# PaoPaoRobot/ygz-slam

Measured on NVIDIA H100. Metric: tracked frames/sec, higher is better.
Workload: dtype u8+f32+f64

## Files before the change

ygz_slam_b200/csrc/align.cu:

```cuda
#include <algorithm>
#include <cstdlib>
#include <mutex>

#include <cooperative_groups.h>

#include "common.cuh"
#include "se3.cuh"
#include "track.cuh"

namespace ygzb {

namespace {

struct LevelImg {
    const uint8_t* d;
    int w, h, pitch;
};

__device__ __forceinline__ LevelImg level_img(const uint8_t* pyr, size_t slot_stride, int slot, const Geometry& g, int L) {
    return LevelImg{pyr + (size_t)slot * slot_stride + g.lv[L].off, g.lv[L].w, g.lv[L].h, g.lv[L].pitch};
}

__device__ void inverse3f(const float H[3][3], float inv[3][3]) {
#define COF(i, j) (H[(i + 1) % 3][(j + 1) % 3] * H[(i + 2) % 3][(j + 2) % 3] - H[(i + 1) % 3][(j + 2) % 3] * H[(i + 2) % 3][(j + 1) % 3])
// ... 524 lines not shown
    cluster.sync();
    if (rank == 0 && tid == 0) {
        const SE3d Tref = se3_from_mat(a.T_ref + 12 * (size_t)prob);
        se3_to_mat(se3_mul(s_T, Tref), a.T_cur + 12 * (size_t)prob);
        a.n_meas_out[prob] = (int32_t)(s_last_nmeas / 16);
    }
}


constexpr int kSA2Threads = 256;
constexpr int kSA2Terms = 21 + 6 + 1;

struct SA2Feat {
    float patch[16], gdx[16], gdy[16];
    double FJ[12];
    double G[3];
    double xyz[3];
    float u, v;
    int ui, vi;
    int state;
    int pad;
};

__device__ __forceinline__ double sa2_rcp(double x) {
    double r;
    asm("rcp.approx.ftz.f64 %0, %1;" : "=d"(r) : "d"(x));
    r = fma(r, fma(-x, r, 1.0), r);
    r = fma(r, fma(-x, r, 1.0), r);
    return r;
}

__device__ bool ldlt_solve6_fast(const double H[6][6], const double b[6], double x[6]) {
    double L[6][6], D[6], rD[6];
    for (int j = 0; j < 6; ++j) {
        double d = H[j][j];
        for (int k = 0; k < j; ++k) d -= L[j][k] * L[j][k] * D[k];
        D[j] = d;
        if (!(fabs(d) > 0)) return false;
        rD[j] = sa2_rcp(fabs(d));
        if (d < 0) rD[j] = -rD[j];
        L[j][j] = 1;
        for (int i = j + 1; i < 6; ++i) {
            double s = H[i][j];
            for (int k = 0; k < j; ++k) s -= L[i][k] * L[j][k] * D[k];
            L[i][j] = s * rD[j];
        }
    }
    double y[6];
    for (int i = 0; i < 6; ++i) {
        double s = b[i];
        for (int k = 0; k < i; ++k) s -= L[i][k] * y[k];
        y[i] = s;
    }
    for (int i = 0; i < 6; ++i) y[i] *= rD[i];
    for (int i = 5; i >= 0; --i) {
        double s = y[i];
        for (int k = i + 1; k < 6; ++k) s -= L[k][i] * x[k];
        x[i] = s;
    }
    return true;
}

// ... 233 lines not shown
    b.cur_slot[j] = job.cur_slot;
    b.n_cand[j] = 0;
    b.c_off[j] = j * b.cap;
    if (j == 0) b.c_off[b.J] = b.J * b.cap;
    if (b.prev) {
        const int r = 2 * job.stream + st.ref_cur[job.stream];
        b.ref_slot[j] = b.job_ref_slot[j];
        b.offsets[j] = j * st.ref_cap;
        if (j == 0) b.offsets[b.J] = b.J * st.ref_cap;
        b.in_off[j] = r * st.ref_cap;
        b.n_feat[j] = st.ref_n[r];
        for (int c = 0; c < 12; ++c) b.T_ref[12 * (size_t)j + c] = b.T_cur[12 * (size_t)j + c] = st.ref_T[12 * (size_t)r + c];
        return;
    }
    const int e = job.stream * st.R + job.entry[job.n_local - 1];
    b.ref_slot[j] = st.kf_slot[e];
    b.offsets[j] = j * st.cells;
    if (j == 0) b.offsets[b.J] = b.J * st.cells;
    b.in_off[j] = e * st.cells;
    b.n_feat[j] = st.kf_n[e];
    for (int c = 0; c < 12; ++c) b.T_ref[12 * (size_t)j + c] = b.T_cur[12 * (size_t)j + c] = (c == 0 || c == 5 || c == 10) ? 1.0 : 0.0;
}

__global__ void track_compose_kernel(TrackStore st, TrackBatch b) {
    const int j = blockIdx.x * blockDim.x + threadIdx.x;
    if (j >= b.J) return;
    const ygzb_track_job job = b.jobs[j];
    if (b.prev) {
        for (int c = 0; c < 12; ++c) b.T_aligned[12 * (size_t)j + c] = b.T_cur[12 * (size_t)j + c];
        return;
    }
    const double* Tk = st.kf_T + 12 * (size_t)(job.stream * st.R + job.entry[job.n_local - 1]);
    const SE3d Trel = se3_from_mat(b.T_cur + 12 * (size_t)j), Tref = se3_from_mat(Tk);
    se3_to_mat(se3_mul(Trel, Tref), b.T_cur + 12 * (size_t)j);
    for (int c = 0; c < 12; ++c) {
        b.T_ref[12 * (size_t)j + c] = Tk[c];
        b.T_aligned[12 * (size_t)j + c] = b.T_cur[12 * (size_t)j + c];
    }
}

__global__ void track_motion_kernel(TrackStore st, TrackBatch b) {
    const int j = blockIdx.x * blockDim.x + threadIdx.x;
    if (j >= b.J) return;
    const ygzb_track_job job = b.jobs[j];
    const double* Tc = b.T_cur + 12 * (size_t)j;
    double inv_ref[12], tcr[12], lg[6];
    mat34_inv(b.T_ref + 12 * (size_t)j, inv_ref);
    mat34_mul(Tc, inv_ref, tcr);
    se3_log(se3_from_mat(tcr), lg);
    double nrm = 0;
    for (int k = 0; k < 6; ++k) nrm += lg[k] * lg[k];
    b.aligned[j] = sqrt(nrm) <= 0.2 ? 1 : 0;
    for (int k = 0; k < job.n_local; ++k) {
        double inv_k[12];
        mat34_inv(st.kf_T + 12 * (size_t)(job.stream * st.R + job.entry[k]), inv_k);
        mat34_mul(Tc, inv_k, b.rel + 12 * ((size_t)j * kTrackMaxLocal + k));
    }
}

__global__ void __launch_bounds__(128) track_project_kernel(const uint8_t* __restrict__ pyr, size_t slot_stride, Geometry g, CamF cam,
                                                            TrackStore st, TrackBatch b) {
    const int j = blockIdx.y, c = blockIdx.x * blockDim.x + threadIdx.x;
    if (c >= b.cap) return;
    const size_t at = (size_t)j * b.cap + c;
    b.cand_ok[at] = 0;
    if (!b.aligned[j]) return;
    const ygzb_track_job job = b.jobs[j];
    const int k = c / st.cells, f = c - k * st.cells;
    if (k >= job.n_local) return;
    const int e = job.stream * st.R + job.entry[k];
    if (f >= st.kf_n[e]) return;
    const double* X = st.kf_pw + 3 * ((size_t)e * st.cells + f);
    const double* T = b.T_cur + 12 * (size_t)j;
    const double x = T[0] * X[0] + T[1] * X[1] + T[2] * X[2] + T[3];
    const double y = T[4] * X[0] + T[5] * X[1] + T[6] * X[2] + T[7];
    const double z = T[8] * X[0] + T[9] * X[1] + T[10] * X[2] + T[11];
    double u = st.fx * x / z + st.cx, v = st.fy * y / z + st.cy;
    if (!(z > 0 && u >= 20 && u < st.W - 20 && v >= 20 && v < st.H - 20)) return;
    atomicAdd(&b.n_cand[j], 1);
    const double eye[12] = {1, 0, 0, 0, 0, 1, 0, 0, 0, 0, 1, 0};
// ... 15 lines not shown
        if (lane >= o) v += u;
    }
    if (lane == 31) s_w[warp] = v;
    __syncthreads();
    if (warp == 0) {
        int w = s_w[lane];
#pragma unroll
        for (int o = 1; o < 32; o <<= 1) {
            const int u = __shfl_up_sync(0xFFFFFFFFu, w, o);
            if (lane >= o) w += u;
        }
        s_w[lane] = w;
        if (lane == 31) s_w[32] = w;
    }
    __syncthreads();
    const int out = v + (warp ? s_w[warp - 1] : 0);
    *total = s_w[32];
    __syncthreads();
    return out;
}

__global__ void __launch_bounds__(1024) track_compact_kernel(TrackStore st, TrackBatch b) {
    __shared__ int s_scan[33];
    __shared__ int s_carry;
    const int j = blockIdx.x, tid = threadIdx.x;
    const ygzb_track_job job = b.jobs[j];
    const int total = job.n_local * st.cells;
    if (tid == 0) s_carry = 0;
    __syncthreads();
    for (int base = 0; base < total; base += 1024) {
        const int c = base + tid;
        const int flag = (c < total && b.cand_ok[(size_t)j * b.cap + c]) ? 1 : 0;
        int chunk_total;
        const int incl = block_scan_1024(flag, s_scan, &chunk_total);
        if (flag) {
            const size_t dst = (size_t)j * b.cap + s_carry + incl - 1;
            const int k = c / st.cells, f = c - k * st.cells;
            const size_t fe = (size_t)(job.stream * st.R + job.entry[k]) * st.cells + f;
            b.c_src[dst] = c;
            b.c_px[2 * dst] = b.cand_px[2 * ((size_t)j * b.cap + c)];
            b.c_px[2 * dst + 1] = b.cand_px[2 * ((size_t)j * b.cap + c) + 1];
            b.c_pw[3 * dst] = st.kf_pw[3 * fe];
            b.c_pw[3 * dst + 1] = st.kf_pw[3 * fe + 1];
            b.c_pw[3 * dst + 2] = st.kf_pw[3 * fe + 2];
        }
        __syncthreads();
        if (tid == 0) s_carry += chunk_total;
        __syncthreads();
    }
    if (tid == 0) b.c_cnt[j] = s_carry;
}

}

size_t sparse_align2_scratch_bytes(int n_problems, int max_features) { return (size_t)n_problems * max_features * sizeof(SA2Feat); }
size_t sparse_align_ws_doubles(int n_problems) { return (size_t)n_problems * 2 * kSparseCluster * (kNormalTerms + 1); }

int launch_align2d(ygzb_frames* f, int n, const int32_t* d_slot, const uint8_t* d_level, const uint8_t* d_ref_border,
                   const uint8_t* d_ref, int n_iter, double* d_uv, uint8_t* d_ok) {
    ygzb_ctx* ctx = f->ctx;
    if (n <= 0) return YGZB_OK;
    ProfScope ps(ctx, kStageAlign2D);
    align2d_kernel<<<(n + 127) / 128, 128, 0, ctx->stream>>>(f->d_pyr, ctx->slot_stride, ctx->geo, n, d_slot, d_level, d_ref_border,
                                                             d_ref, n_iter, d_uv, d_ok);
    YGZB_LAUNCHED(ctx);
    return YGZB_OK;
}

int launch_align1d(ygzb_frames* f, int n, const int32_t* d_slot, const uint8_t* d_level, const float* d_dir, const uint8_t* d_ref_border,
                   const uint8_t* d_ref, int n_iter, double* d_uv, uint8_t* d_ok, double* d_hinv) {
    ygzb_ctx* ctx = f->ctx;
    if (n <= 0) return YGZB_OK;
    ProfScope ps(ctx, kStageAlign2D);
// ... 145 lines not shown
    a.max_level = 2;
    a.min_level = 0;
    a.n_iter = 30;
    a.eps = 1e-6;
    a.n_meas_out = b.n_meas;
    a.iters_out = nullptr;
    a.ref_patch = b.ref_patch;
    a.gdx = b.gdx;
    a.gdy = b.gdy;
    a.frame_jac = b.frame_jac;
    a.visible = b.visible;
    a.ws = b.sparse_ws;
    a.feat_scratch = nullptr;
    a.feat_stride = 0;
    if (gen1) return launch_sparse_align1(ctx, a, b.J, sparse_cluster);
    return launch_sparse_align2(ctx, a, b.J, sparse_cluster, b.sa2_scratch, sparse_align2_scratch_bytes(1, feat_cap));
}

int launch_track_chain_mid(ygzb_frames* f, const TrackStore& st, const TrackBatch& b) {
    ygzb_ctx* ctx = f->ctx;
    if (b.J <= 0) return YGZB_OK;
    {
        ProfScope ps(ctx, kStageOther);
        track_compose_kernel<<<(b.J + 63) / 64, 64, 0, ctx->stream>>>(st, b);
        YGZB_LAUNCHED(ctx);
    }
    {
        ProfScope ps(ctx, kStageOther);
        track_motion_kernel<<<(b.J + 63) / 64, 64, 0, ctx->stream>>>(st, b);
        YGZB_LAUNCHED(ctx);
    }
    {
        const CamF cam{ctx->prm.fx, ctx->prm.fy, ctx->prm.cx, ctx->prm.cy};
        ProfScope ps(ctx, kStageProjectAlign);
        track_project_kernel<<<dim3((unsigned)((b.cap + 127) / 128), (unsigned)b.J), 128, 0, ctx->stream>>>(f->d_pyr, ctx->slot_stride, ctx->geo,
                                                                                                          cam, st, b);
        YGZB_LAUNCHED(ctx);
    }
    {
        ProfScope ps(ctx, kStageOther);
        track_compact_kernel<<<(unsigned)b.J, 1024, 0, ctx->stream>>>(st, b);
        YGZB_LAUNCHED(ctx);
    }
    return YGZB_OK;
}

}
```

ygz_slam_b200/csrc/ba.cu:

```cuda
#include <algorithm>
#include <cstdlib>
#include <cstring>
#include <exception>
#include <mutex>
#include <utility>
#include <vector>

#include <cooperative_groups.h>

#include "ba2.cuh"
#include "common.cuh"
#include "se3.cuh"
#include "track.cuh"

namespace ygzb {

namespace {

constexpr int kBAThreads = 256;
constexpr int kMaxFreePoses = 16;
constexpr int kMaxPoses = 64;

struct BAArgs {
    const int32_t *kf_off, *pt_off, *obs_off;
// ... 846 lines not shown
    double* T_cw;
    uint8_t* inlier;
    double* depth;
    int32_t* n_inlier;
    uint8_t* enable;
    double* ws;
    float fx, fy, cx, cy;
    int stage_k;
};

constexpr int kPoseThreads = 256;
constexpr int kPoseCluster = 8;
constexpr int kPoseRed = 32;

__device__ bool cholesky6(double A[36], double y[6]) {
    double rd[6];
#pragma unroll
    for (int j = 0; j < 6; ++j) {
        double d = A[j * 6 + j];
#pragma unroll
        for (int k = 0; k < j; ++k) d -= A[j * 6 + k] * A[j * 6 + k] * A[k * 6 + k];
        if (!(d > 0)) return false;
        A[j * 6 + j] = d;
        rd[j] = 1.0 / d;
#pragma unroll
        for (int i = j + 1; i < 6; ++i) {
            double s = A[i * 6 + j];
#pragma unroll
            for (int k = 0; k < j; ++k) s -= A[i * 6 + k] * A[j * 6 + k] * A[k * 6 + k];
            A[i * 6 + j] = s * rd[j];
        }
    }
#pragma unroll
    for (int i = 0; i < 6; ++i) {
        double s = y[i];
#pragma unroll
        for (int k = 0; k < i; ++k) s -= A[i * 6 + k] * y[k];
        y[i] = s;
    }
#pragma unroll
    for (int i = 0; i < 6; ++i) y[i] *= rd[i];
#pragma unroll
    for (int i = 5; i >= 0; --i) {
        double s = y[i];
#pragma unroll
        for (int k = i + 1; k < 6; ++k) s -= A[k * 6 + i] * y[k];
        y[i] = s;
    }
    return true;
}

__global__ void __launch_bounds__(kPoseThreads) pose_only_kernel(const PoseOnlyArgs a) {
    namespace cg = cooperative_groups;
    cg::cluster_group cluster = cg::this_cluster();
    extern __shared__ double s_pts[];
    __shared__ double s_red[kPoseThreads / 32][kPoseRed];
    __shared__ double s_pub[4][kPoseRed];
    __shared__ double s_pose[6], s_cand[6], s_scale[6], s_sum[kPoseRed];
    __shared__ double s_R[9], s_dR[27], s_Rpose[6];
    const int rank = (int)cluster.block_rank(), C = (int)cluster.num_blocks();
    const int prob = blockIdx.x / C, tid = threadIdx.x, lane = tid & 31, warp = tid >> 5;
    const int CT = C * kPoseThreads, ct = rank * kPoseThreads + tid;
    const int i0 = a.offsets[prob], n = a.counts ? a.counts[prob] : a.offsets[prob + 1] - i0;
    const double fx = a.fx, fy = a.fy, cx = a.cx, cy = a.cy;
    const int K = (n + CT - 1) / CT;
    const bool staged = K <= a.stage_k && K <= 32;
    unsigned en_mask = 0;
    int slot = 0;

    auto finish_reduce = [&](int cnt) {
        __syncthreads();
        if (tid < cnt) {
            double s = 0;
            for (int w = 0; w < kPoseThreads / 32; ++w) s += s_red[w][tid];
            s_pub[slot][tid] = s;
        }
        cluster.sync();
        if (tid < cnt) {
            double s = 0;
            for (int r = 0; r < C; ++r) s += cluster.map_shared_rank(&s_pub[slot][0], r)[tid];
            s_sum[tid] = s;
        }
        slot = (slot + 1) & 3;
        __syncthreads();
    };
    auto reduce_few = [&](const double* part, int cnt) {
        for (int t = 0; t < cnt; ++t) {
            const double v = warp_sum(part[t]);
            if (lane == 0) s_red[warp][t] = v;
        }
        finish_reduce(cnt);
    };
    auto reduce32 = [&](double* part) {
        s_red[warp][lane] = warp_reduce_scatter<32>(part, lane);
        finish_reduce(32);
    };
    auto rotation_of = [&](const double* pose) {
        bool same = true;
        for (int k = 0; k < 6; ++k) same = same && s_Rpose[k] == pose[k];
        if (same) return;
        __syncthreads();
        if (tid < 3) {
            double col[3], dcol[3][3];
            const double aa[3] = {pose[3], pose[4], pose[5]};
            rotate_basis(aa, tid, col, dcol);
            for (int j = 0; j < 3; ++j) {
                s_R[3 * j + tid] = col[j];
                for (int m = 0; m < 3; ++m) s_dR[3 * (3 * j + tid) + m] = dcol[j][m];
            }
        }
        if (tid >= 32 && tid < 38) s_Rpose[tid - 32] = pose[tid - 32];
        __syncthreads();
    };
    auto point = [&](int k, double* X, double* o) {
        if (staged) {
#pragma unroll
            for (int c = 0; c < 3; ++c) X[c] = s_pts[(k * 5 + c) * kPoseThreads + tid];
            o[0] = s_pts[(k * 5 + 3) * kPoseThreads + tid];
            o[1] = s_pts[(k * 5 + 4) * kPoseThreads + tid];
        } else {
            const size_t i = (size_t)(i0 + ct + k * CT);
#pragma unroll
            for (int c = 0; c < 3; ++c) X[c] = a.pw[3 * i + c];
            o[0] = (a.px[2 * i] - cx) / fx;
            o[1] = (a.px[2 * i + 1] - cy) / fy;
        }
    };
    auto enabled = [&](int k) { return staged ? (en_mask >> k & 1u) != 0 : a.enable[i0 + ct + k * CT] != 0; };
    auto eval_normal = [&](const double* pose) {
        rotation_of(pose);
        double part[32];
#pragma unroll
        for (int t = 0; t < 32; ++t) part[t] = 0;
        const double t0 = pose[0], t1 = pose[1], t2 = pose[2];
        for (int k = 0; k < K; ++k) {
            if (ct + k * CT >= n || !enabled(k)) continue;
            double X[3], o[2];
            point(k, X, o);
            const double p2 = s_R[6] * X[0] + s_R[7] * X[1] + s_R[8] * X[2] + t2;
            if (p2 < 0) {
                part[28] += 1;
                continue;
            }
            const double p0 = s_R[0] * X[0] + s_R[1] * X[1] + s_R[2] * X[2] + t0, p1 = s_R[3] * X[0] + s_R[4] * X[1] + s_R[5] * X[2] + t1;
            const double inv = 1.0 / p2, q0 = p0 * inv, q1 = p1 * inv, r0 = o[0] - q0, r1 = o[1] - q1;
            double dp[3][3];
#pragma unroll
            for (int j = 0; j < 3; ++j)
#pragma unroll
                for (int m = 0; m < 3; ++m)
                    dp[j][m] = s_dR[3 * (3 * j) + m] * X[0] + s_dR[3 * (3 * j + 1) + m] * X[1] + s_dR[3 * (3 * j + 2) + m] * X[2];
            double j0[6], j1[6];
            j0[0] = -inv; j0[1] = 0.0; j0[2] = q0 * inv;
            j1[0] = 0.0; j1[1] = -inv; j1[2] = q1 * inv;
#pragma unroll
            for (int m = 0; m < 3; ++m) {
                j0[3 + m] = -(dp[0][m] - q0 * dp[2][m]) * inv;
                j1[3 + m] = -(dp[1][m] - q1 * dp[2][m]) * inv;
            }
            int t = 0;
#pragma unroll
            for (int r = 0; r < 6; ++r) {
#pragma unroll
                for (int c = r; c < 6; ++c) part[t++] += j0[r] * j0[c] + j1[r] * j1[c];
            }
#pragma unroll
            for (int q = 0; q < 6; ++q) part[21 + q] += j0[q] * r0 + j1[q] * r1;
            part[27] += r0 * r0 + r1 * r1;
        }
        reduce32(part);
    };

    SE3d T = se3_from_mat(a.T_cw + 12 * (size_t)prob);
    double backup[6];
    {
        double th;
        const V3d rl = so3_log(T.q, &th);
        backup[0] = T.t.x; backup[1] = T.t.y; backup[2] = T.t.z; backup[3] = rl.x; backup[4] = rl.y; backup[5] = rl.z;
    }
    for (int k = 0; k < K; ++k) {
        const int i = ct + k * CT;
        if (i >= n) break;
        a.enable[i0 + i] = 1;
        a.inlier[i0 + i] = 1;
        a.depth[i0 + i] = -1;
        if (staged) {
            en_mask |= 1u << k;
#pragma unroll
            for (int c = 0; c < 3; ++c) s_pts[(k * 5 + c) * kPoseThreads + tid] = a.pw[3 * (size_t)(i0 + i) + c];
            s_pts[(k * 5 + 3) * kPoseThreads + tid] = (a.px[2 * (size_t)(i0 + i)] - cx) / fx;
            s_pts[(k * 5 + 4) * kPoseThreads + tid] = (a.px[2 * (size_t)(i0 + i) + 1] - cy) / fy;
        }
    }
    if (tid < 6) s_Rpose[tid] = __longlong_as_double(0x7FF8000000000000LL);
    __syncthreads();
    int cntInlier = 0;
    for (int round = 0; round < 4; ++round) {
        if (tid < 6) s_pose[tid] = backup[tid];
        __syncthreads();
        eval_normal(s_pose);
        bool run = !(s_sum[28] > 0);
        double cost = 0.5 * s_sum[27];
        if (run) {
            if (tid < 6) {
                int t = 0;
                for (int r = 0; r < tid; ++r) t += 6 - r;
                s_scale[tid] = 1.0 / (1.0 + sqrt(s_sum[t]));
            }
            double gmax = 0;
            for (int k = 0; k < 6; ++k) gmax = fmax(gmax, fabs(s_sum[21 + k]));
            if (gmax <= 1e-10) run = false;
        }
        __syncthreads();
        double radius = 1e4, decrease_factor = 2.0;
        double U[27];
        for (int t = 0; t < 27; ++t) U[t] = s_sum[t];
        __syncthreads();
        for (int iter = 0; run && iter < 50; ++iter) {
            double A[36], g[6], y[6];
            {
                int t = 0;
                for (int r = 0; r < 6; ++r)
                    for (int c = r; c < 6; ++c) {
                        A[r * 6 + c] = A[c * 6 + r] = U[t++] * s_scale[r] * s_scale[c];
                    }
                for (int k = 0; k < 6; ++k) g[k] = U[21 + k] * s_scale[k];
            }
            double An[36];
            for (int t = 0; t < 36; ++t) An[t] = A[t];
            for (int k = 0; k < 6; ++k) {
                const double d = fmin(fmax(A[k * 6 + k], 1e-6), 1e32);
                An[k * 6 + k] += d / radius;
                y[k] = -g[k];
            }
            bool step_ok = cholesky6(An, y);
            double model_cost_change = 0;
            if (step_ok) {
                double yg = 0, yAy = 0;
                for (int r = 0; r < 6; ++r) {
                    yg += y[r] * g[r];
                    double s = 0;
                    for (int c = 0; c < 6; ++c) s += A[r * 6 + c] * y[c];
                    yAy += y[r] * s;
                }
                model_cost_change = -yg - 0.5 * yAy;
                step_ok = model_cost_change > 0;
            }
            bool accepted = false;
            if (step_ok) {
                double step_norm = 0, x_norm = 0;
                if (tid < 6) s_cand[tid] = s_pose[tid] + y[tid] * s_scale[tid];
                for (int k = 0; k < 6; ++k) {
                    const double d = y[k] * s_scale[k];
                    step_norm += d * d;
                    x_norm += s_pose[k] * s_pose[k];
                }
                step_norm = sqrt(step_norm);
                x_norm = sqrt(x_norm);
                __syncthreads();
                eval_normal(s_cand);
                const double new_cost = 0.5 * s_sum[27];
                if (!(s_sum[28] > 0)) {
                    const double relative_decrease = (cost - new_cost) / model_cost_change;
                    if (relative_decrease > 1e-3) {
                        accepted = true;
                        if (step_norm <= 1e-8 * (x_norm + 1e-8)) break;
                        const double cost_change = cost - new_cost;
                        __syncthreads();
                        if (tid < 6) s_pose[tid] = s_cand[tid];
                        __syncthreads();
                        const double old_cost = cost;
                        cost = new_cost;
                        if (fabs(cost_change) <= 1e-6 * old_cost) break;
                        double gmax = 0;
                        for (int k = 0; k < 6; ++k) gmax = fmax(gmax, fabs(s_sum[21 + k]));
                        for (int t = 0; t < 27; ++t) U[t] = s_sum[t];
                        __syncthreads();
                        if (gmax <= 1e-10) break;
                        radius = radius / fmax(1.0 / 3.0, 1.0 - pow(2.0 * relative_decrease - 1.0, 3));
                        radius = fmin(1e16, radius);
                        decrease_factor = 2.0;
                    }
                }
            }
            if (!accepted) {
                radius = radius / decrease_factor;
                decrease_factor *= 2.0;
                if (radius < 1e-32) break;
            }
            __syncthreads();
        }
        __syncthreads();
        double cnt = 0;
        for (int k = 0; k < K; ++k) {
            const int i = ct + k * CT;
            if (i >= n) break;
            const double* X = a.pw + 3 * (size_t)(i0 + i);
            const V3d pc = transform(T, V3d{X[0], X[1], X[2]});
            const double u = fx * pc.x / pc.z + cx, v = fy * pc.y / pc.z + cy;
            const double dx = u - a.px[2 * (size_t)(i0 + i)], dy = v - a.px[2 * (size_t)(i0 + i) + 1];
            const double error2 = dx * dx + dy * dy;
            if (error2 > (double)5.991f) {
                a.inlier[i0 + i] = 0;
                a.enable[i0 + i] = 0;
                en_mask &= ~(1u << (k & 31));
            } else {
                a.depth[i0 + i] = pc.z;
                a.inlier[i0 + i] = 1;
                a.enable[i0 + i] = 1;
                en_mask |= 1u << (k & 31);
                cnt += 1;
            }
        }
        reduce_few(&cnt, 1);
        cntInlier = (int)s_sum[0];
        if (cntInlier < 10) break;
        double th;
        T.q = so3_exp(V3d{s_pose[3], s_pose[4], s_pose[5]}, &th);
        T.t = V3d{s_pose[0], s_pose[1], s_pose[2]};
        __syncthreads();
    }
    cluster.sync();
    if (rank == 0 && tid == 0) {
        se3_to_mat(T, a.T_cw + 12 * (size_t)prob);
        a.n_inlier[prob] = cntInlier;
    }
}

}

size_t pose_only_ws_doubles(int n_problems) { return (size_t)n_problems * 4 * kPoseCluster * kPoseRed; }

static int pose_only_stage_k(int max_points, int cluster) {
    static std::once_flag once;
    static int max_k = 0;
    std::call_once(once, [] {
        int dev = 0, optin = 0;
        cudaGetDevice(&dev);
        cudaDeviceGetAttribute(&optin, cudaDevAttrMaxSharedMemoryPerBlockOptin, dev);
        const int budget = std::max(0, optin - 8 * 1024);
        cudaFuncSetAttribute(pose_only_kernel, cudaFuncAttributeMaxDynamicSharedMemorySize, budget);
        max_k = std::min(32, budget / (int)(5 * kPoseThreads * sizeof(double)));
    });
    const int k = (std::max(max_points, 1) + cluster * kPoseThreads - 1) / (cluster * kPoseThreads);
    return k <= max_k ? k : 0;
}

int launch_pose_only_dev(ygzb_ctx* ctx, int n_problems, const int32_t* d_offsets, const int32_t* d_counts, const double* d_pw,
                         const double* d_px, double* d_T_cw, uint8_t* d_inlier, double* d_depth, int32_t* d_n_inlier, uint8_t* d_enable,
                         double* d_ws, int cluster, int max_points) {
    if (n_problems <= 0) return YGZB_OK;
    PoseOnlyArgs a;
    a.offsets = d_offsets; a.counts = d_counts; a.pw = d_pw; a.px = d_px; a.T_cw = d_T_cw; a.inlier = d_inlier; a.depth = d_depth;
    a.n_inlier = d_n_inlier; a.enable = d_enable; a.ws = d_ws;
    a.fx = ctx->prm.fx; a.fy = ctx->prm.fy; a.cx = ctx->prm.cx; a.cy = ctx->prm.cy;
    cluster = std::max(1, std::min(cluster, kPoseCluster));
    a.stage_k = pose_only_stage_k(max_points, cluster);
    cudaLaunchConfig_t cfg{};
    cfg.gridDim = dim3((unsigned)(n_problems * cluster));
    cfg.blockDim = dim3(kPoseThreads);
    cfg.dynamicSmemBytes = (size_t)a.stage_k * 5 * kPoseThreads * sizeof(double);
    cfg.stream = ctx->stream;
    cudaLaunchAttribute attr[1];
    attr[0].id = cudaLaunchAttributeClusterDimension;
    attr[0].val.clusterDim.x = cluster;
    attr[0].val.clusterDim.y = 1;
    attr[0].val.clusterDim.z = 1;
    cfg.attrs = attr;
    cfg.numAttrs = 1;
    ProfScope ps(ctx, kStagePoseOnly);
    YGZB_CUDA(ctx, cudaLaunchKernelEx(&cfg, pose_only_kernel, a));
    YGZB_LAUNCHED(ctx);
    return YGZB_OK;
}

}

using namespace ygzb;

namespace {
template <typename T>
int h2d(ygzb_ctx* ctx, T* dst, const T* src, size_t count) {
    if (!count) return YGZB_OK;
    return check_cuda(ctx, cudaMemcpyAsync(dst, src, count * sizeof(T), cudaMemcpyHostToDevice, ctx->stream), "H2D");
}
template <typename T>
int d2h(ygzb_ctx* ctx, T* dst, const T* src, size_t count) {
    if (!count) return YGZB_OK;
    return check_cuda(ctx, cudaMemcpyAsync(dst, src, count * sizeof(T), cudaMemcpyDeviceToHost, ctx->stream), "D2H");
}
#define TRY(x)                          \
    do {                                \
        int _rc = (x);                  \
        if (_rc != YGZB_OK) return _rc; \
    } while (0)
}
// ... 507 lines not shown
        };
        put(d_off, offsets, (P + 1) * 4);
        put(d_pw, pt_world, 3 * N * 8);
        put(d_px, px, 2 * N * 8);
        put(a.T_cw, T_cw, 12 * P * 8);
        YGZB_CUDA(ctx, cudaMemcpyAsync(buf, stage, in_bytes, cudaMemcpyHostToDevice, ctx->stream));
    }
    {
        int max_points = 0;
        for (size_t q = 0; q < P; ++q) max_points = std::max(max_points, offsets[q + 1] - offsets[q]);
        a.stage_k = pose_only_stage_k(max_points, kPoseCluster);
        cudaLaunchConfig_t cfg{};
        cfg.gridDim = dim3((unsigned)(n_problems * kPoseCluster));
        cfg.blockDim = dim3(kPoseThreads);
        cfg.dynamicSmemBytes = (size_t)a.stage_k * 5 * kPoseThreads * sizeof(double);
        cfg.stream = ctx->stream;
        cudaLaunchAttribute attr[1];
        attr[0].id = cudaLaunchAttributeClusterDimension;
        attr[0].val.clusterDim.x = kPoseCluster;
        attr[0].val.clusterDim.y = 1;
        attr[0].val.clusterDim.z = 1;
        cfg.attrs = attr;
        cfg.numAttrs = 1;
        ProfScope ps(ctx, kStagePoseOnly);
        YGZB_CUDA(ctx, cudaLaunchKernelEx(&cfg, pose_only_kernel, a));
    }
    YGZB_LAUNCHED(ctx);
    TRY(d2h(ctx, T_cw, a.T_cw, 12 * P));
    TRY(d2h(ctx, inlier, a.inlier, N));
    TRY(d2h(ctx, depth, a.depth, N));
    TRY(d2h(ctx, n_inlier, a.n_inlier, P));
    YGZB_CUDA(ctx, cudaStreamSynchronize(ctx->stream));
    return YGZB_OK;
}

}
```

ygz_slam_b200/csrc/ba2.cu:

```cuda
#include <algorithm>
#include <cstdlib>
#include <cstring>
#include <mutex>

#include <cooperative_groups.h>

#include "ba2.cuh"
#include "common.cuh"
#include "se3.cuh"

namespace ygzb {

namespace {

namespace cg = cooperative_groups;

constexpr int kT = kBA2Threads;
constexpr int kW = kT / 32;
constexpr int kPairW = 42;
constexpr int kPoseW = 27;

__device__ __forceinline__ double warp_sum(double v) {
#pragma unroll
    for (int o = 16; o > 0; o >>= 1) v += __shfl_down_sync(0xFFFFFFFFu, v, o);
// ... 22 lines not shown
    __syncthreads();
    v0 = s_tmp[kW];
    v1 = s_tmp[2 * kW + 1];
}

__device__ double block_max(double v, double* s_tmp) {
    const int lane = threadIdx.x & 31, warp = threadIdx.x >> 5;
#pragma unroll
    for (int o = 16; o > 0; o >>= 1) v = fmax(v, __shfl_down_sync(0xFFFFFFFFu, v, o));
    __syncthreads();
    if (lane == 0) s_tmp[warp] = v;
    __syncthreads();
    if (warp == 0) {
        double t = lane < kW ? s_tmp[lane] : 0.0;
#pragma unroll
        for (int o = 16; o > 0; o >>= 1) t = fmax(t, __shfl_down_sync(0xFFFFFFFFu, t, o));
        if (lane == 0) s_tmp[kW] = t;
    }
    __syncthreads();
    return s_tmp[kW];
}

constexpr int kCtaSolveMinDim = 24;

__device__ __forceinline__ double fast_rcp(double x) {
    double r;
    asm("rcp.approx.ftz.f64 %0, %1;" : "=d"(r) : "d"(x));
    r = fma(r, fma(-x, r, 1.0), r);
    r = fma(r, fma(-x, r, 1.0), r);
    return r;
}

__device__ __forceinline__ SE3d pose_from_g2o(const double* est) {
    const double v[6] = {est[3], est[4], est[5], est[0], est[1], est[2]};
    return se3_exp(v);
}

struct Jac {
    double l0[3], l1[3];
    double p0[6], p1[6];
};
__device__ __forceinline__ void pose_jac(double x, double y, double iz, double fx, double fy, double* p0, double* p1) {
    const double iz2 = iz * iz;
    p0[0] = x * y * iz2 * fx; p0[1] = -(1.0 + x * x * iz2) * fx; p0[2] = y * iz * fx;
    p0[3] = -iz * fx; p0[4] = 0.0; p0[5] = x * iz2 * fx;
    p1[0] = (1.0 + y * y * iz2) * fy; p1[1] = -x * y * iz2 * fy; p1[2] = -x * iz * fy;
    p1[3] = 0.0; p1[4] = -iz * fy; p1[5] = y * iz2 * fy;
}
__device__ __forceinline__ void point_jac(double x, double y, double iz_pos, double fx, double fy, const double* R ,
                                          double* l0, double* l1) {
    const double iz = -iz_pos;
    const double t02 = x * iz * fx, t12 = y * iz * fy;
#pragma unroll
    for (int c = 0; c < 3; ++c) {
// ... 1046 lines not shown
```

ygz_slam_b200/csrc/common.cuh:

```cuda
#pragma once

#include <cuda_runtime.h>
#include <stdint.h>
#include <stdio.h>
#include <string.h>

#include <vector>

#include "../../include/ygz_b200.h"

namespace ygzb {

constexpr int kMaxLevels = YGZB_MAX_LEVELS;

constexpr int kTileW = 80;
constexpr int kTileH = 40;

struct LevelGeom {
    int w, h, pitch;
    unsigned off;
};

struct Geometry {
    LevelGeom lv[kMaxLevels];
// ... 137 lines not shown
struct Carver {
    uint8_t* base;
    size_t off = 0;
    explicit Carver(void* p) : base(static_cast<uint8_t*>(p)) {}
    template <typename T>
    T* take(size_t count) {
        off = (off + 255) & ~(size_t)255;
        T* r = base ? reinterpret_cast<T*>(base + off) : nullptr;
        off += count * sizeof(T);
        return r;
    }
    size_t bytes() const { return off + 256; }
};

__device__ __forceinline__ unsigned float_orderable(float f) {
    unsigned u = __float_as_uint(f);
    return (u & 0x80000000u) ? ~u : (u | 0x80000000u);
}
__device__ __forceinline__ float orderable_float(unsigned o) {
    unsigned u = (o & 0x80000000u) ? (o & 0x7FFFFFFFu) : ~o;
    return __uint_as_float(u);
}

__device__ __forceinline__ double select_f64(bool c, double a, double b) {
    double r;
    asm("{\n\t.reg .pred p;\n\tsetp.ne.u32 p, %1, 0;\n\tselp.f64 %0, %2, %3, p;\n\t}" : "=d"(r) : "r"((unsigned)c), "d"(a), "d"(b));
    return r;
}

template <int N, int M = N>
__device__ __forceinline__ double warp_reduce_scatter(double* v, int lane) {
    static_assert((N == 16 || N == 32) && 2 * M > N && M <= N, "warp_reduce_scatter: N = 16 or 32 values, at most N / 2 of them padding");
#pragma unroll
    for (int s = 0; s < 5; ++s) {
        const int n = (N >> 1) >> s, off = 16 >> s;
        if (n == 0) {
            v[0] += __shfl_xor_sync(0xFFFFFFFFu, v[0], off);
            continue;
        }
        const bool up = (lane & off) != 0;
#pragma unroll
        for (int i = 0; i < N / 2; ++i) {
            if (i >= n) continue;
            const double hi = i + n < M ? v[i + n] : 0.0;
            const double keep = select_f64(up, hi, v[i]);
            const double send = select_f64(up, v[i], hi);
// ... 8 lines not shown
```

Measured before the change: 30280.

## Streamline pose-only LM loop, fuse track pose kernels, single-pass compaction

Merges the track compose and motion kernels into one launch. Rewrites candidate compaction so each thread scans a contiguous chunk with a bitmask and a single block scan, replacing the multi-pass chunked scan. In the pose-only optimizer it skips re-optimisation when the inlier set is unchanged, computes the candidate rotation inline so the evaluation pass can skip its own rotation update, drops redundant barriers, replaces pow with cubing, and uses a fast reciprocal in the Cholesky solve. It also adds an env-gated clock64 debug profiling variant. The risks are small numerical differences from the approximate reciprocal and the changed iteration control.

```diff
diff --git a/ygz_slam_b200/csrc/align.cu b/ygz_slam_b200/csrc/align.cu
--- a/ygz_slam_b200/csrc/align.cu
+++ b/ygz_slam_b200/csrc/align.cu
@@ -570,14 +570,6 @@
     int pad;
 };
 
-__device__ __forceinline__ double sa2_rcp(double x) {
-    double r;
-    asm("rcp.approx.ftz.f64 %0, %1;" : "=d"(r) : "d"(x));
-    r = fma(r, fma(-x, r, 1.0), r);
-    r = fma(r, fma(-x, r, 1.0), r);
-    return r;
-}
-
 __device__ bool ldlt_solve6_fast(const double H[6][6], const double b[6], double x[6]) {
     double L[6][6], D[6], rD[6];
     for (int j = 0; j < 6; ++j) {
@@ -585,7 +577,7 @@
         for (int k = 0; k < j; ++k) d -= L[j][k] * L[j][k] * D[k];
         D[j] = d;
         if (!(fabs(d) > 0)) return false;
-        rD[j] = sa2_rcp(fabs(d));
+        rD[j] = fast_rcp(fabs(d));
         if (d < 0) rD[j] = -rD[j];
         L[j][j] = 1;
         for (int i = j + 1; i < 6; ++i) {
@@ -865,10 +857,7 @@
     for (int c = 0; c < 12; ++c) b.T_ref[12 * (size_t)j + c] = b.T_cur[12 * (size_t)j + c] = (c == 0 || c == 5 || c == 10) ? 1.0 : 0.0;
 }
 
-__global__ void track_compose_kernel(TrackStore st, TrackBatch b) {
-    const int j = blockIdx.x * blockDim.x + threadIdx.x;
-    if (j >= b.J) return;
-    const ygzb_track_job job = b.jobs[j];
+__device__ void track_compose(const TrackStore& st, const TrackBatch& b, int j, const ygzb_track_job& job) {
     if (b.prev) {
         for (int c = 0; c < 12; ++c) b.T_aligned[12 * (size_t)j + c] = b.T_cur[12 * (size_t)j + c];
         return;
@@ -882,10 +871,7 @@
     }
 }
 
-__global__ void track_motion_kernel(TrackStore st, TrackBatch b) {
-    const int j = blockIdx.x * blockDim.x + threadIdx.x;
-    if (j >= b.J) return;
-    const ygzb_track_job job = b.jobs[j];
+__device__ void track_motion(const TrackStore& st, const TrackBatch& b, int j, const ygzb_track_job& job) {
     const double* Tc = b.T_cur + 12 * (size_t)j;
     double inv_ref[12], tcr[12], lg[6];
     mat34_inv(b.T_ref + 12 * (size_t)j, inv_ref);
@@ -899,6 +885,14 @@
         mat34_inv(st.kf_T + 12 * (size_t)(job.stream * st.R + job.entry[k]), inv_k);
         mat34_mul(Tc, inv_k, b.rel + 12 * ((size_t)j * kTrackMaxLocal + k));
     }
+}
+
+__global__ void track_pose_kernel(TrackStore st, TrackBatch b) {
+    const int j = blockIdx.x * blockDim.x + threadIdx.x;
+    if (j >= b.J) return;
+    const ygzb_track_job job = b.jobs[j];
+    track_compose(st, b, j, job);
+    track_motion(st, b, j, job);
 }
 
 __global__ void __launch_bounds__(128) track_project_kernel(const uint8_t* __restrict__ pyr, size_t slot_stride, Geometry g, CamF cam,
@@ -960,33 +954,34 @@
 
 __global__ void __launch_bounds__(1024) track_compact_kernel(TrackStore st, TrackBatch b) {
     __shared__ int s_scan[33];
-    __shared__ int s_carry;
     const int j = blockIdx.x, tid = threadIdx.x;
     const ygzb_track_job job = b.jobs[j];
     const int total = job.n_local * st.cells;
-    if (tid == 0) s_carry = 0;
-    __syncthreads();
-    for (int base = 0; base < total; base += 1024) {
-        const int c = base + tid;
-        const int flag = (c < total && b.cand_ok[(size_t)j * b.cap + c]) ? 1 : 0;
-        int chunk_total;
-        const int incl = block_scan_1024(flag, s_scan, &chunk_total);
-        if (flag) {
-            const size_t dst = (size_t)j * b.cap + s_carry + incl - 1;
-            const int k = c / st.cells, f = c - k * st.cells;
-            const size_t fe = (size_t)(job.stream * st.R + job.entry[k]) * st.cells + f;
-            b.c_src[dst] = c;
-            b.c_px[2 * dst] = b.cand_px[2 * ((size_t)j * b.cap + c)];
-            b.c_px[2 * dst + 1] = b.cand_px[2 * ((size_t)j * b.cap + c) + 1];
-            b.c_pw[3 * dst] = st.kf_pw[3 * fe];
-            b.c_pw[3 * dst + 1] = st.kf_pw[3 * fe + 1];
-            b.c_pw[3 * dst + 2] = st.kf_pw[3 * fe + 2];
-        }
-        __syncthreads();
-        if (tid == 0) s_carry += chunk_total;
-        __syncthreads();
-    }
-    if (tid == 0) b.c_cnt[j] = s_carry;
+    const int per = (total + 1023) / 1024;
+    const uint8_t* ok = b.cand_ok + (size_t)j * b.cap;
+    unsigned mask = 0;
+    for (int q = 0; q < per; ++q) {
+        const int c = tid * per + q;
+        if (c < total && ok[c]) mask |= 1u << q;
+    }
+    int n_total;
+    const int mine = __popc(mask);
+    size_t dst = (size_t)j * b.cap + (block_scan_1024(mine, s_scan, &n_total) - mine);
+    while (mask) {
+        const int q = __ffs(mask) - 1;
+        mask &= mask - 1;
+        const int c = tid * per + q;
+        const int k = c / st.cells, f = c - k * st.cells;
+        const size_t fe = (size_t)(job.stream * st.R + job.entry[k]) * st.cells + f;
+        b.c_src[dst] = c;
+        b.c_px[2 * dst] = b.cand_px[2 * ((size_t)j * b.cap + c)];
+        b.c_px[2 * dst + 1] = b.cand_px[2 * ((size_t)j * b.cap + c) + 1];
+        b.c_pw[3 * dst] = st.kf_pw[3 * fe];
+        b.c_pw[3 * dst + 1] = st.kf_pw[3 * fe + 1];
+        b.c_pw[3 * dst + 2] = st.kf_pw[3 * fe + 2];
+        ++dst;
+    }
+    if (tid == 0) b.c_cnt[j] = n_total;
 }
 
 }
@@ -1178,12 +1173,7 @@
     if (b.J <= 0) return YGZB_OK;
     {
         ProfScope ps(ctx, kStageOther);
-        track_compose_kernel<<<(b.J + 63) / 64, 64, 0, ctx->stream>>>(st, b);
-        YGZB_LAUNCHED(ctx);
-    }
-    {
-        ProfScope ps(ctx, kStageOther);
-        track_motion_kernel<<<(b.J + 63) / 64, 64, 0, ctx->stream>>>(st, b);
+        track_pose_kernel<<<(b.J + 63) / 64, 64, 0, ctx->stream>>>(st, b);
         YGZB_LAUNCHED(ctx);
     }
     {
diff --git a/ygz_slam_b200/csrc/ba.cu b/ygz_slam_b200/csrc/ba.cu
--- a/ygz_slam_b200/csrc/ba.cu
+++ b/ygz_slam_b200/csrc/ba.cu
@@ -892,7 +892,7 @@
         for (int k = 0; k < j; ++k) d -= A[j * 6 + k] * A[j * 6 + k] * A[k * 6 + k];
         if (!(d > 0)) return false;
         A[j * 6 + j] = d;
-        rd[j] = 1.0 / d;
+        rd[j] = fast_rcp(d);
 #pragma unroll
         for (int i = j + 1; i < 6; ++i) {
             double s = A[i * 6 + j];
@@ -920,6 +920,10 @@
     return true;
 }
 
+enum PoseDbgPhase { kPdRotation = 0, kPdPoints, kPdCtaReduce, kPdClusterGather, kPdSolve, kPdClassify, kPdOther, kPdPhases };
+constexpr int kPoseDbgWords = 16;
+
+template <bool kDebug>
 __global__ void __launch_bounds__(kPoseThreads) pose_only_kernel(const PoseOnlyArgs a) {
     namespace cg = cooperative_groups;
     cg::cluster_group cluster = cg::this_cluster();
@@ -928,6 +932,7 @@
     __shared__ double s_pub[4][kPoseRed];
     __shared__ double s_pose[6], s_cand[6], s_scale[6], s_sum[kPoseRed];
     __shared__ double s_R[9], s_dR[27], s_Rpose[6];
+    __shared__ long long s_dbg[kDebug ? kPoseDbgWords : 1];
     const int rank = (int)cluster.block_rank(), C = (int)cluster.num_blocks();
     const int prob = blockIdx.x / C, tid = threadIdx.x, lane = tid & 31, warp = tid >> 5;
     const int CT = C * kPoseThreads, ct = rank * kPoseThreads + tid;
@@ -937,6 +942,26 @@
     const bool staged = K <= a.stage_k && K <= 32;
     unsigned en_mask = 0;
     int slot = 0;
+    if constexpr (kDebug) {
+        if (tid == 0) {
+            for (int q = 0; q < kPoseDbgWords - 1; ++q) s_dbg[q] = 0;
+            s_dbg[12] = s_dbg[15] = clock64();
+        }
+    }
+    auto tick = [&](int ph) {
+        if constexpr (kDebug) {
+            if (tid == 0) {
+                const long long now = clock64();
+                s_dbg[ph] += now - s_dbg[15];
+                s_dbg[15] = now;
+            }
+        }
+    };
+    auto count = [&](int q) {
+        if constexpr (kDebug) {
+            if (tid == 0) s_dbg[q] += 1;
+        }
+    };
 
     auto finish_reduce = [&](int cnt) {
         __syncthreads();
@@ -945,14 +970,20 @@
             for (int w = 0; w < kPoseThreads / 32; ++w) s += s_red[w][tid];
             s_pub[slot][tid] = s;
         }
+        tick(kPdCtaReduce);
         cluster.sync();
         if (tid < cnt) {
+            double v[kPoseCluster];
+#pragma unroll
+            for (int r = 0; r < kPoseCluster; ++r) v[r] = r < C ? cluster.map_shared_rank(&s_pub[slot][0], r)[tid] : 0.0;
             double s = 0;
-            for (int r = 0; r < C; ++r) s += cluster.map_shared_rank(&s_pub[slot][0], r)[tid];
+#pragma unroll
+            for (int r = 0; r < kPoseCluster; ++r) s += v[r];
             s_sum[tid] = s;
         }
         slot = (slot + 1) & 3;
         __syncthreads();
+        tick(kPdClusterGather);
     };
     auto reduce_few = [&](const double* part, int cnt) {
         for (int t = 0; t < cnt; ++t) {
@@ -965,22 +996,27 @@
         s_red[warp][lane] = warp_reduce_scatter<32>(part, lane);
         finish_reduce(32);
     };
+    auto rotation_column = [&](const double aa[3]) {
+        double col[3], dcol[3][3];
+        rotate_basis(aa, tid, col, dcol);
+        for (int j = 0; j < 3; ++j) {
+            s_R[3 * j + tid] = col[j];
+            for (int m = 0; m < 3; ++m) s_dR[3 * (3 * j + tid) + m] = dcol[j][m];
+        }
+    };
     auto rotation_of = [&](const double* pose) {
+        tick(kPdOther);
         bool same = true;
         for (int k = 0; k < 6; ++k) same = same && s_Rpose[k] == pose[k];
         if (same) return;
         __syncthreads();
         if (tid < 3) {
-            double col[3], dcol[3][3];
             const double aa[3] = {pose[3], pose[4], pose[5]};
-            rotate_basis(aa, tid, col, dcol);
-            for (int j = 0; j < 3; ++j) {
-                s_R[3 * j + tid] = col[j];
-                for (int m = 0; m < 3; ++m) s_dR[3 * (3 * j + tid) + m] = dcol[j][m];
-            }
+            rotation_column(aa);
         }
         if (tid >= 32 && tid < 38) s_Rpose[tid - 32] = pose[tid - 32];
         __syncthreads();
+        tick(kPdRotation);
     };
     auto point = [&](int k, double* X, double* o) {
         if (staged) {
@@ -997,8 +1033,10 @@
         }
     };
     auto enabled = [&](int k) { return staged ? (en_mask >> k & 1u) != 0 : a.enable[i0 + ct + k * CT] != 0; };
-    auto eval_normal = [&](const double* pose) {
-        rotation_of(pose);
+    auto eval_normal = [&](const double* pose, bool have_rotation) {
+        count(7);
+        if (!have_rotation) rotation_of(pose);
+        tick(kPdOther);
         double part[32];
 #pragma unroll
         for (int t = 0; t < 32; ++t) part[t] = 0;
@@ -1038,6 +1076,7 @@
             for (int q = 0; q < 6; ++q) part[21 + q] += j0[q] * r0 + j1[q] * r1;
             part[27] += r0 * r0 + r1 * r1;
         }
+        tick(kPdPoints);
         reduce32(part);
     };
 
@@ -1065,106 +1104,119 @@
     if (tid < 6) s_Rpose[tid] = __longlong_as_double(0x7FF8000000000000LL);
     __syncthreads();
     int cntInlier = 0;
+    bool same_set = false;
     for (int round = 0; round < 4; ++round) {
-        if (tid < 6) s_pose[tid] = backup[tid];
+        if (!same_set) {
+            if (tid < 6) s_pose[tid] = backup[tid];
+            __syncthreads();
+            eval_normal(s_pose, false);
+            bool run = !(s_sum[28] > 0);
+            double cost = 0.5 * s_sum[27];
+            if (run) {
+                if (tid < 6) {
+                    int t = 0;
+                    for (int r = 0; r < tid; ++r) t += 6 - r;
+                    s_scale[tid] = 1.0 / (1.0 + sqrt(s_sum[t]));
+                }
+                double gmax = 0;
+                for (int k = 0; k < 6; ++k) gmax = fmax(gmax, fabs(s_sum[21 + k]));
+                if (gmax <= 1e-10) run = false;
+            }
+            __syncthreads();
+            double radius = 1e4, decrease_factor = 2.0;
+            double U[27];
+            for (int t = 0; t < 27; ++t) U[t] = s_sum[t];
+            __syncthreads();
+            for (int iter = 0; run && iter < 50; ++iter) {
+                count(8 + round);
+                tick(kPdOther);
+                double A[36], g[6], y[6];
+                {
+                    int t = 0;
+                    for (int r = 0; r < 6; ++r)
+                        for (int c = r; c < 6; ++c) {
+                            A[r * 6 + c] = A[c * 6 + r] = U[t++] * s_scale[r] * s_scale[c];
+                        }
+                    for (int k = 0; k < 6; ++k) g[k] = U[21 + k] * s_scale[k];
+                }
+                double An[36];
+                for (int t = 0; t < 36; ++t) An[t] = A[t];
+                for (int k = 0; k < 6; ++k) {
+                    const double d = fmin(fmax(A[k * 6 + k], 1e-6), 1e32);
+                    An[k * 6 + k] += d / radius;
+                    y[k] = -g[k];
+                }
+                bool step_ok = cholesky6(An, y);
+                double model_cost_change = 0;
+                if (step_ok) {
+                    double yg = 0, yAy = 0;
+                    for (int r = 0; r < 6; ++r) {
+                        yg += y[r] * g[r];
+                        double s = 0;
+                        for (int c = 0; c < 6; ++c) s += A[r * 6 + c] * y[c];
+                        yAy += y[r] * s;
+                    }
+                    model_cost_change = -yg - 0.5 * yAy;
+                    step_ok = model_cost_change > 0;
+                }
+                tick(kPdSolve);
+                bool accepted = false;
+                if (step_ok) {
+                    double step_norm = 0, x_norm = 0;
+                    if (tid < 6) s_cand[tid] = fma(y[tid], s_scale[tid], s_pose[tid]);
+                    if (tid < 3) {
+                        double aa[3];
+#pragma unroll
+                        for (int m = 0; m < 3; ++m) aa[m] = fma(y[3 + m], s_scale[3 + m], s_pose[3 + m]);
+                        rotation_column(aa);
+                    }
+                    if (tid >= 32 && tid < 38) s_Rpose[tid - 32] = fma(y[tid - 32], s_scale[tid - 32], s_pose[tid - 32]);
+                    for (int k = 0; k < 6; ++k) {
+                        const double d = y[k] * s_scale[k];
+                        step_norm += d * d;
+                        x_norm += s_pose[k] * s_pose[k];
+                    }
+                    step_norm = sqrt(step_norm);
+                    x_norm = sqrt(x_norm);
+                    __syncthreads();
+                    eval_normal(s_cand, true);
+                    const double new_cost = 0.5 * s_sum[27];
+                    if (!(s_sum[28] > 0)) {
+                        const double relative_decrease = (cost - new_cost) / model_cost_change;
+                        if (relative_decrease > 1e-3) {
+                            accepted = true;
+                            if (step_norm <= 1e-8 * (x_norm + 1e-8)) break;
+                            const double cost_change = cost - new_cost;
+                            if (tid < 6) s_pose[tid] = s_cand[tid];
+                            const double old_cost = cost;
+                            cost = new_cost;
+                            if (fabs(cost_change) <= 1e-6 * old_cost) break;
+                            double gmax = 0;
+                            for (int k = 0; k < 6; ++k) gmax = fmax(gmax, fabs(s_sum[21 + k]));
+                            for (int t = 0; t < 27; ++t) U[t] = s_sum[t];
+                            if (gmax <= 1e-10) break;
+                            const double rho = 2.0 * relative_decrease - 1.0;
+                            radius = radius / fmax(1.0 / 3.0, 1.0 - rho * rho * rho);
+                            radius = fmin(1e16, radius);
+                            decrease_factor = 2.0;
+                        }
+                    }
+                }
+                if (!accepted) {
+                    radius = radius / decrease_factor;
+                    decrease_factor *= 2.0;
+                    if (radius < 1e-32) break;
+                }
+                __syncthreads();
+            }
+        }
         __syncthreads();
-        eval_normal(s_pose);
-        bool run = !(s_sum[28] > 0);
-        double cost = 0.5 * s_sum[27];
-        if (run) {
-            if (tid < 6) {
-                int t = 0;
-                for (int r = 0; r < tid; ++r) t += 6 - r;
-                s_scale[tid] = 1.0 / (1.0 + sqrt(s_sum[t]));
-            }
-            double gmax = 0;
-            for (int k = 0; k < 6; ++k) gmax = fmax(gmax, fabs(s_sum[21 + k]));
-            if (gmax <= 1e-10) run = false;
-        }
-        __syncthreads();
-        double radius = 1e4, decrease_factor = 2.0;
-        double U[27];
-        for (int t = 0; t < 27; ++t) U[t] = s_sum[t];
-        __syncthreads();
-        for (int iter = 0; run && iter < 50; ++iter) {
-            double A[36], g[6], y[6];
-            {
-                int t = 0;
-                for (int r = 0; r < 6; ++r)
-                    for (int c = r; c < 6; ++c) {
-                        A[r * 6 + c] = A[c * 6 + r] = U[t++] * s_scale[r] * s_scale[c];
-                    }
-                for (int k = 0; k < 6; ++k) g[k] = U[21 + k] * s_scale[k];
-            }
-            double An[36];
-            for (int t = 0; t < 36; ++t) An[t] = A[t];
-            for (int k = 0; k < 6; ++k) {
-                const double d = fmin(fmax(A[k * 6 + k], 1e-6), 1e32);
-                An[k * 6 + k] += d / radius;
-                y[k] = -g[k];
-            }
-            bool step_ok = cholesky6(An, y);
-            double model_cost_change = 0;
-            if (step_ok) {
-                double yg = 0, yAy = 0;
-                for (int r = 0; r < 6; ++r) {
-                    yg += y[r] * g[r];
-                    double s = 0;
-                    for (int c = 0; c < 6; ++c) s += A[r * 6 + c] * y[c];
-                    yAy += y[r] * s;
-                }
-                model_cost_change = -yg - 0.5 * yAy;
-                step_ok = model_cost_change > 0;
-            }
-            bool accepted = false;
-            if (step_ok) {
-                double step_norm = 0, x_norm = 0;
-                if (tid < 6) s_cand[tid] = s_pose[tid] + y[tid] * s_scale[tid];
-                for (int k = 0; k < 6; ++k) {
-                    const double d = y[k] * s_scale[k];
-                    step_norm += d * d;
-                    x_norm += s_pose[k] * s_pose[k];
-                }
-                step_norm = sqrt(step_norm);
-                x_norm = sqrt(x_norm);
-                __syncthreads();
-                eval_normal(s_cand);
-                const double new_cost = 0.5 * s_sum[27];
-                if (!(s_sum[28] > 0)) {
-                    const double relative_decrease = (cost - new_cost) / model_cost_change;
-                    if (relative_decrease > 1e-3) {
-                        accepted = true;
-                        if (step_norm <= 1e-8 * (x_norm + 1e-8)) break;
-                        const double cost_change = cost - new_cost;
-                        __syncthreads();
-                        if (tid < 6) s_pose[tid] = s_cand[tid];
-                        __syncthreads();
-                        const double old_cost = cost;
-                        cost = new_cost;
-                        if (fabs(cost_change) <= 1e-6 * old_cost) break;
-                        double gmax = 0;
-                        for (int k = 0; k < 6; ++k) gmax = fmax(gmax, fabs(s_sum[21 + k]));
-                        for (int t = 0; t < 27; ++t) U[t] = s_sum[t];
-                        __syncthreads();
-                        if (gmax <= 1e-10) break;
-                        radius = radius / fmax(1.0 / 3.0, 1.0 - pow(2.0 * relative_decrease - 1.0, 3));
-                        radius = fmin(1e16, radius);
-                        decrease_factor = 2.0;
-                    }
-                }
-            }
-            if (!accepted) {
-                radius = radius / decrease_factor;
-                decrease_factor *= 2.0;
-                if (radius < 1e-32) break;
-            }
-            __syncthreads();
-        }
-        __syncthreads();
-        double cnt = 0;
+        tick(kPdOther);
+        double cls[2] = {0, 0};
         for (int k = 0; k < K; ++k) {
             const int i = ct + k * CT;
             if (i >= n) break;
+            const bool was = enabled(k);
             const double* X = a.pw + 3 * (size_t)(i0 + i);
             const V3d pc = transform(T, V3d{X[0], X[1], X[2]});
             const double u = fx * pc.x / pc.z + cx, v = fy * pc.y / pc.z + cy;
@@ -1174,16 +1226,20 @@
                 a.inlier[i0 + i] = 0;
                 a.enable[i0 + i] = 0;
                 en_mask &= ~(1u << (k & 31));
+                if (was) cls[1] += 1;
             } else {
                 a.depth[i0 + i] = pc.z;
                 a.inlier[i0 + i] = 1;
                 a.enable[i0 + i] = 1;
                 en_mask |= 1u << (k & 31);
-                cnt += 1;
-            }
-        }
-        reduce_few(&cnt, 1);
+                cls[0] += 1;
+                if (!was) cls[1] += 1;
+            }
+        }
+        tick(kPdClassify);
+        reduce_few(cls, 2);
         cntInlier = (int)s_sum[0];
+        same_set = !(s_sum[1] > 0);
         if (cntInlier < 10) break;
         double th;
         T.q = so3_exp(V3d{s_pose[3], s_pose[4], s_pose[5]}, &th);
@@ -1194,6 +1250,15 @@
     if (rank == 0 && tid == 0) {
         se3_to_mat(T, a.T_cw + 12 * (size_t)prob);
         a.n_inlier[prob] = cntInlier;
+    }
+    if constexpr (kDebug) {
+        tick(kPdOther);
+        if (rank == 0 && tid == 0) {
+            s_dbg[12] = clock64() - s_dbg[12];
+            s_dbg[13] = n;
+            s_dbg[14] = K;
+            for (int q = 0; q < kPoseDbgWords - 1; ++q) a.ws[(size_t)prob * 4 * kPoseCluster * kPoseRed + q] = (double)s_dbg[q];
+        }
     }
 }
 
@@ -1209,11 +1274,41 @@
         cudaGetDevice(&dev);
         cudaDeviceGetAttribute(&optin, cudaDevAttrMaxSharedMemoryPerBlockOptin, dev);
         const int budget = std::max(0, optin - 8 * 1024);
-        cudaFuncSetAttribute(pose_only_kernel, cudaFuncAttributeMaxDynamicSharedMemorySize, budget);
+        cudaFuncSetAttribute(pose_only_kernel<false>, cudaFuncAttributeMaxDynamicSharedMemorySize, budget);
         max_k = std::min(32, budget / (int)(5 * kPoseThreads * sizeof(double)));
     });
     const int k = (std::max(max_points, 1) + cluster * kPoseThreads - 1) / (cluster * kPoseThreads);
     return k <= max_k ? k : 0;
+}
+
+static int launch_pose_kernel(ygzb_ctx* ctx, const cudaLaunchConfig_t& cfg, const PoseOnlyArgs& a, int n_problems) {
+    const bool debug = getenv("YGZB_POSE_DEBUG") != nullptr;
+    {
+        ProfScope ps(ctx, kStagePoseOnly);
+        if (debug) {
+            static std::once_flag once;
+            std::call_once(once, [] {
+                int dev = 0, optin = 0;
+                cudaGetDevice(&dev);
+                cudaDeviceGetAttribute(&optin, cudaDevAttrMaxSharedMemoryPerBlockOptin, dev);
+                cudaFuncSetAttribute(pose_only_kernel<true>, cudaFuncAttributeMaxDynamicSharedMemorySize, std::max(0, optin - 8 * 1024));
+            });
+            YGZB_CUDA(ctx, cudaLaunchKernelEx(&cfg, pose_only_kernel<true>, a));
+        } else {
+            YGZB_CUDA(ctx, cudaLaunchKernelEx(&cfg, pose_only_kernel<false>, a));
+        }
+    }
+    YGZB_LAUNCHED(ctx);
+    if (debug) {
+        double h[kPoseDbgWords] = {};
+        YGZB_CUDA(ctx, cudaStreamSynchronize(ctx->stream));
+        YGZB_CUDA(ctx, cudaMemcpy(h, a.ws, sizeof(double) * (kPoseDbgWords - 1), cudaMemcpyDeviceToHost));
+        fprintf(stderr, "[pose_only] problems=%d cluster=%u n=%.0f K=%.0f evals=%.0f iters=%.0f,%.0f,%.0f,%.0f cycles=%.0f rotation=%.0f "
+                        "points=%.0f cta_reduce=%.0f cluster_gather=%.0f solve=%.0f classify=%.0f other=%.0f\n",
+                n_problems, cfg.attrs[0].val.clusterDim.x, h[13], h[14], h[7], h[8], h[9], h[10], h[11], h[12], h[kPdRotation],
+                h[kPdPoints], h[kPdCtaReduce], h[kPdClusterGather], h[kPdSolve], h[kPdClassify], h[kPdOther]);
+    }
+    return YGZB_OK;
 }
 
 int launch_pose_only_dev(ygzb_ctx* ctx, int n_problems, const int32_t* d_offsets, const int32_t* d_counts, const double* d_pw,
@@ -1238,10 +1333,7 @@
     attr[0].val.clusterDim.z = 1;
     cfg.attrs = attr;
     cfg.numAttrs = 1;
-    ProfScope ps(ctx, kStagePoseOnly);
-    YGZB_CUDA(ctx, cudaLaunchKernelEx(&cfg, pose_only_kernel, a));
-    YGZB_LAUNCHED(ctx);
-    return YGZB_OK;
+    return launch_pose_kernel(ctx, cfg, a, n_problems);
 }
 
 }
@@ -1795,10 +1887,9 @@
         attr[0].val.clusterDim.z = 1;
         cfg.attrs = attr;
         cfg.numAttrs = 1;
-        ProfScope ps(ctx, kStagePoseOnly);
-        YGZB_CUDA(ctx, cudaLaunchKernelEx(&cfg, pose_only_kernel, a));
-    }
-    YGZB_LAUNCHED(ctx);
+        const int rc = launch_pose_kernel(ctx, cfg, a, n_problems);
+        if (rc != YGZB_OK) return rc;
+    }
     TRY(d2h(ctx, T_cw, a.T_cw, 12 * P));
     TRY(d2h(ctx, inlier, a.inlier, N));
     TRY(d2h(ctx, depth, a.depth, N));
diff --git a/ygz_slam_b200/csrc/ba2.cu b/ygz_slam_b200/csrc/ba2.cu
--- a/ygz_slam_b200/csrc/ba2.cu
+++ b/ygz_slam_b200/csrc/ba2.cu
@@ -68,14 +68,6 @@
 }
 
 constexpr int kCtaSolveMinDim = 24;
-
-__device__ __forceinline__ double fast_rcp(double x) {
-    double r;
-    asm("rcp.approx.ftz.f64 %0, %1;" : "=d"(r) : "d"(x));
-    r = fma(r, fma(-x, r, 1.0), r);
-    r = fma(r, fma(-x, r, 1.0), r);
-    return r;
-}
 
 __device__ __forceinline__ SE3d pose_from_g2o(const double* est) {
     const double v[6] = {est[3], est[4], est[5], est[0], est[1], est[2]};
diff --git a/ygz_slam_b200/csrc/common.cuh b/ygz_slam_b200/csrc/common.cuh
--- a/ygz_slam_b200/csrc/common.cuh
+++ b/ygz_slam_b200/csrc/common.cuh
@@ -183,6 +183,14 @@
     return __uint_as_float(u);
 }
 
+__device__ __forceinline__ double fast_rcp(double x) {
+    double r;
+    asm("rcp.approx.ftz.f64 %0, %1;" : "=d"(r) : "d"(x));
+    r = fma(r, fma(-x, r, 1.0), r);
+    r = fma(r, fma(-x, r, 1.0), r);
+    return r;
+}
+
 __device__ __forceinline__ double select_f64(bool c, double a, double b) {
     double r;
     asm("{\n\t.reg .pred p;\n\tsetp.ne.u32 p, %1, 0;\n\tselp.f64 %0, %2, %3, p;\n\t}" : "=d"(r) : "r"((unsigned)c), "d"(a), "d"(b));
```

New measurement: 31830, median of 6. 5.1% higher.
